# konstantineder/montecarlo-risk-engine

Measured on AMD Instinct MI355X. Metric: path-steps/sec at 1M paths x 250 steps; PV/CVA rel-error vs CPU ref, higher is better.
Workload: dtype f64

## Files before the change

### montecarlo-risk-engine_amd/csrc/kf_lean.hip

```cpp
#include <cstdlib>
#include <map>
#include <utility>

#include "kf_common.h"

namespace {

template <int NSLOT, int PPL>
__device__ __forceinline__ void lean_date_cva(const FastDateCvaLds* __restrict__ rp, const double (&reg)[PPL][2 * NSLOT], double (&cva)[PPL],
                                              const double* __restrict__ etab)
{
    const mcx_expq_coef ec = mcx_expq_load(mcx_region_zero());
    const FastDateCvaLds r = *rp;
    double xe[2 * PPL], ev[2 * PPL];
#pragma unroll
    for (int q = 0; q < PPL; ++q) {
        xe[2 * q] = fma(r.m_s1, reg[q][FDC_S_REG], fma(r.m_n1, reg[q][FDC_NI_REG], r.m_c0));
        xe[2 * q + 1] = fma(r.c_c1, reg[q][FDC_C_REG], r.c_c0);
    }
    mcx_exp_tab_n<2 * PPL>(xe, ev, etab, ec);
#pragma unroll
    for (int q = 0; q < PPL; ++q) {
        const double x = fma(r.x_d, reg[q][FDC_X_REG], r.x_a);
        double p = 0.0;
// ... 121 lines not shown
        const double r2 = fma(ed[q], -2.0 * 6.93147180559945309417e-01, tc[q].y) + fma(s * s, p, s);
        const double r = mcx_sqrt_gp(r2);
        const double sn = fma(sc[q].x, pc[q], sc[q].y * ps[q]);
        const double cs = fma(-sc[q].x, ps[q], sc[q].y * pc[q]);
        z0[q] = r * cs;
        z1[q] = r * sn;
        top = w1[q] > top ? w1[q] : top;
    }
    return top == 0xffffffffu;
}

#define MCX_LEAN_WAVES 4
template <int NSLOT, int NZ, bool INJECT, int SIG, int PPL, bool SIMULATE, int DK = 0>
__global__ __launch_bounds__(MCX_BLOCK, MCX_LEAN_WAVES) void kf_lean(const FusedArgs)
{
    static_assert(DK == 0 || (SIG == SIG_VAS_CIR_E && SIMULATE && !INJECT), "the cva-date kernel simulates the Vasicek + CIR++ signature");
    constexpr int NREG = 2 * NSLOT;
    constexpr int TILE = MCX_BLOCK * PPL;
    extern __shared__ double lds[];
    KArgs& a0 = kargs_region(0);
    const int n_rec = a0.n_rec;
    const int64_t n = a0.k1.n;
    for (int q = threadIdx.x; q < 9 * n_rec; q += MCX_BLOCK) lds[q] = 0.0;
    FastDateCvaLds* const dlds = (FastDateCvaLds*)(lds + ((9 * n_rec + 1) & ~1));
    if constexpr (DK != 0) {
        const FastDateCva* __restrict__ dc = a0.cva_dates;
        const double* __restrict__ cf = a0.coeffs;
        const int n_dates = a0.n_dates;
        for (int q = threadIdx.x; q < 16 * n_dates; q += MCX_BLOCK) {
            const int t = q >> 4, e = q & 15;
            double v;
            if (e < FDC_HEAD) {
                v = ((const double*)(dc + t))[e];
            } else {
                const int off = e < FDC_HEAD + 3 ? dc[t].coeff_off0 : dc[t].coeff_off1;
                v = off >= 0 ? cf[off + (e - FDC_HEAD) % 3] : 0.0;
            }
            ((double*)dlds)[q] = v;
        }
    }
    constexpr int BMB = SIG == SIG_VAS_CIR_E ? 10 : 7;
    constexpr int BM = (INJECT || !SIMULATE) ? 0 : MCX_BM_LDS_DOUBLES_B(BMB);
    __shared__ double tab_lds[BM + MCX_EXP_LDS_DOUBLES];
    const double* tab = nullptr;
    const double* etab = tab_lds + BM;
    mcx_exp_tab_load(tab_lds + BM);
    if (BM) { mcx_bm_load<BMB>(tab_lds); tab = tab_lds; }
    __syncthreads();
    const int64_t tiles = (n + TILE - 1) / TILE;
    double n_block = 0.0;

    for (int64_t tile = blockIdx.x; tile < tiles; tile += gridDim.x) {
        const bool first_tile = tile == (int64_t)blockIdx.x;
        int64_t i[PPL];
        bool live[PPL];
        uint64_t path[PPL];
        double reg[PPL][NREG];
        double cfs[PPL], cva[PPL];
        int est[PPL];
        int n_init, n_steps;
        {
            KArgs& a = kargs_region(mcx_region_zero());
            const auto& k = a.k1;
#pragma unroll
            for (int q = 0; q < PPL; ++q) {
                const int64_t i_raw = tile * TILE + q * MCX_BLOCK + threadIdx.x;
                live[q] = i_raw < n;
                i[q] = live[q] ? i_raw : n - 1;
                path[q] = k.path_offset + (uint64_t)i[q];
                sim_init_state<NSLOT, SIG>(k, reg[q]);
                cfs[q] = 0.0; cva[q] = 0.0;
                est[q] = a.init_state[0];
            }
            const int64_t rest = n - tile * TILE;
            n_block += (double)(rest < TILE ? rest : TILE);
            n_init = k.n_initial_store; n_steps = k.n_steps;
        }
        if (SIMULATE) {
        int step = 0, t_init = 0;
#pragma unroll 1
        while (true) {
            const bool init = t_init < n_init;
            if (!init && step >= n_steps) break;
            int st = init ? t_init : -1;
            t_init += init ? 1 : 0;
            {
                const int zr0 = mcx_region_zero();
                const auto& k = kargs_region(zr0).k1;
                const uint64_t seed = k.seed;
                const mcx_bm_coef bc = mcx_bm_coef_load(zr0);
                const mcx_bm_vconst vc = mcx_bm_vconst_make<BMB>(bc);
                uint32_t path_hi = 0;
                CvaDrawConst dc = {};
                if constexpr (DK == 1) { path_hi = ((const MCX_KONST uint32_t*)&k.path_offset)[1]; dc = cva_draw_const_make(); }
#pragma unroll 1
                while (st < 0 && step < n_steps) {
                    if constexpr (SIG == SIG_GENERIC) {
#pragma unroll
                        for (int q = 0; q < PPL; ++q) sim_substep<NSLOT, NZ, INJECT, SIG, BMB, true>(k, step, path[q], i[q], reg[q], tab, seed, bc, &vc);
                        st = ldk(&k.steps[step].store_idx);
                    } else {
                        double zz[PPL][NZ], uu[PPL];
                        bool rare = false;
                        const StepData<NSLOT, NZ> sdat = sim_step_load<NSLOT, NZ, SIG>(k, step);
                        __builtin_amdgcn_sched_barrier(0);
                        if constexpr (INJECT) {
#pragma unroll
                            for (int q = 0; q < PPL; ++q) sim_draw<NZ, true, SIG, BMB>(k, step, path[q], i[q], zz[q], uu[q], tab, seed, bc, &vc);
                        } else if constexpr (DK == 1) {
// ... 52 lines not shown
            load_row(n_dates > 1 ? 1 : 0, bufb);
#pragma unroll 1
            for (int t = 0; t < n_dates; t += 2) {
                lean_date<NSLOT, SIG, PPL, false>(t, i, live, first_tile, lds, reg, cfs, cva, est, etab);
                if (t + 2 < n_dates) load_row(t + 2, reg);
                if (t + 1 < n_dates) {
                    lean_date<NSLOT, SIG, PPL, false>(t + 1, i, live, first_tile, lds, bufb, cfs, cva, est, etab);
                    if (t + 3 < n_dates) load_row(t + 3, bufb);
                }
            }
        }
        {
            KArgs& a = kargs_region(mcx_region_zero());
#pragma unroll
            for (int q = 0; q < PPL; ++q) if (a.cfs && live[q]) a.cfs[i[q]] = cfs[q];
            if (a.rec_pv[0] >= 0) lean_record<PPL>(cfs, live, a.rec_pv[0], n_rec, first_tile, lds);
            if (a.rec_cva[0] >= 0) {
                const double lgd = a.lgd[0];
                double cc[PPL];
#pragma unroll
                for (int q = 0; q < PPL; ++q) cc[q] = cva[q] * lgd;
                lean_record<PPL>(cc, live, a.rec_cva[0], n_rec, first_tile, lds);
            }
        }
    }
    __syncthreads();
    for (int r = threadIdx.x; r < n_rec; r += MCX_BLOCK) {
        double s1 = 0.0, s2 = 0.0;
        for (int w = 0; w < 4; ++w) { s1 += lds[n_rec + (w * n_rec + r) * 2]; s2 += lds[n_rec + (w * n_rec + r) * 2 + 1]; }
        double* dst = a0.partials + ((int64_t)blockIdx.x * n_rec + r) * 4;
        dst[0] = n_block; dst[1] = lds[r]; dst[2] = s1; dst[3] = s2;
    }
}

template <int NSLOT, int NZ, int SIG, int PPL>
int launch_lean_shape(const FusedArgs& a, int full_steps, int n_cu, bool inject, bool simulate, hipStream_t s)
{
// ... 20 lines not shown
    if (!simulate) {
        auto kern = kf_lean<NSLOT, NZ, false, SIG, PPL, false>;
        grid = sized(residency(kern, lds));
        hipLaunchKernelGGL(kern, dim3(grid), dim3(MCX_BLOCK), lds, s, a);
    } else if (inject) {
        auto kern = kf_lean<NSLOT, NZ, true, SIG, PPL, true>;
        grid = sized(residency(kern, lds));
        hipLaunchKernelGGL(kern, dim3(grid), dim3(MCX_BLOCK), lds, s, a);
    } else {
        auto kern = kf_lean<NSLOT, NZ, false, SIG, PPL, true>;
        const int64_t resident = residency(kern, lds);
        if constexpr (SIG == SIG_VAS_CIR_E) {
            auto kern_cva = kf_lean<NSLOT, NZ, false, SIG, 2, true, 1>;
            auto kern_cva_thin = kf_lean<NSLOT, NZ, false, SIG, PPL, true, 2>;
            const bool one_high_word = ((a.k1.path_offset + (uint64_t)(a.k1.n - 1)) >> 32) == (a.k1.path_offset >> 32);
            if (a.cva_dates && one_high_word) {
                grid = sized(resident);
                if (PPL == 2 && grid >= resident) {
                    if (residency(kern_cva, lds_cva) >= resident) {
                        hipLaunchKernelGGL(kern_cva, dim3(grid), dim3(MCX_BLOCK), lds_cva, s, a);
                        return grid;
                    }
                } else if (residency(kern_cva_thin, lds_cva) >= resident) {
                    hipLaunchKernelGGL(kern_cva_thin, dim3(grid), dim3(MCX_BLOCK), lds_cva, s, a);
                    return grid;
                }
            }
        }
        grid = sized(resident);
        FusedArgs g = a;
        g.k1.n_steps = full_steps;
// ... 40 lines not shown
```

### montecarlo-risk-engine_amd/csrc/mcx_math.h

```cpp
#pragma once

__device__ const double MCX_EXP_C[14] __attribute__((aligned(64))) = {1.00000000000000000e+00, 1.00000000000000000e+00, 5.00000000000000000e-01, 1.66666666666666657e-01, 4.16666666666666644e-02, 8.33333333333333322e-03, 1.38888888888888894e-03, 1.98412698412698413e-04, 2.48015873015873016e-05, 2.75573192239858925e-06, 2.75573192239858883e-07, 2.50521083854417202e-08, 2.08767569878681002e-09, 1.60590438368216133e-10};
__device__ const double MCX_SIN_C[10] = {3.14159265358979312e+00, -5.16771278004997026e+00, 2.55016403987734552e+00, -5.99264529320792105e-01, 8.21458866111282326e-02, -7.37043094571435044e-03, 4.66302805767612554e-04, -2.19153534478302173e-05, 7.95205400147551261e-07, -2.29484289972698730e-08};
__device__ const double MCX_COS_C[10] = {1.00000000000000000e+00, -4.93480220054467900e+00, 4.05871212641676848e+00, -1.33526276885458950e+00, 2.35330630358893206e-01, -2.58068913900140612e-02, 1.92957430940392314e-03, -1.04638104924845705e-04, 4.30306958703294729e-06, -1.38789524622137714e-07};
__device__ const double MCX_LOG_C[7] = {6.666666666666735130e-01, 3.999999999940941908e-01, 2.857142874366239149e-01, 2.222219843214978396e-01, 1.818357216161805012e-01, 1.531383769920937332e-01, 1.479819860511658591e-01};

__device__ __forceinline__ int mcx_region_zero()
{
    int z;
    asm volatile("s_mov_b32 %0, 0" : "=s"(z));
    return z;
}
__device__ __forceinline__ uint32_t mcx_region_copy(uint32_t v)
{
    uint32_t o;
    asm volatile("s_mov_b32 %0, %1" : "=s"(o) : "s"(v));
    return o;
}

struct mcx_exp_coef { double c[14]; };
__device__ __forceinline__ mcx_exp_coef mcx_exp_load(int z = 0)
{
    return ldk_struct((const mcx_exp_coef*)(MCX_EXP_C + z));
}
// ... 104 lines not shown

__device__ __forceinline__ double mcx_sqrt_gp(double a)
{
    const double y = __builtin_amdgcn_rsq(a);
    const double g = a * y;
    const double h = 0.5 * y;
    return fma(g, fma(-h, g, 0.5), g);
}

#include "mcx_tables.h"
#define MCX_BM_LDS_DOUBLES_B(BMB) (4 << (BMB))
#define MCX_BM_LDS_DOUBLES MCX_BM_LDS_DOUBLES_B(7)
template <int BMB> struct mcx_bm_shape;
template <> struct mcx_bm_shape<7> {
    static constexpr int LOG_TERMS = 6, TRIG_TERMS = 3;
    static __device__ __forceinline__ double log_src(int q) { return MCX_LOG_TAB[q]; }
    static __device__ __forceinline__ double trig_src(int q) { return MCX_TRIG_TAB[q]; }
};
template <> struct mcx_bm_shape<10> {
    static constexpr int LOG_TERMS = 4, TRIG_TERMS = 2;
    static __device__ __forceinline__ double log_src(int q) { return MCX_LOG_TAB_L[q]; }
    static __device__ __forceinline__ double trig_src(int q) { return MCX_TRIG_TAB_L[q]; }
};

__device__ const double MCX_BM_C[12] __attribute__((aligned(64))) = {0.25, (1.0 / 3.0) * 0.25, 0.03125, 0.2 * 0.0625, (1.0 / 6.0) * 0.03125, (1.0 / 7.0) * 0.015625,
                                                                     -1.0 / 6.0, 1.0 / 120.0, -1.0 / 5040.0, -0.5, 1.0 / 24.0, -1.0 / 720.0};
struct mcx_bm_coef { double c[12]; };
__device__ __forceinline__ mcx_bm_coef mcx_bm_coef_load(int z = 0)
{
    return ldk_struct((const mcx_bm_coef*)(MCX_BM_C + z));
}

struct mcx_bm_vconst {
    double c54;
    double s53, s32;
    double log_head;
    double sin_head, cos_head;
    double trig_off;
};
__device__ __forceinline__ double mcx_opaque_v(double x) { asm volatile("" : "+v"(x)); return x; }
__device__ __forceinline__ double mcx_opaque_s(double x) { asm volatile("" : "+s"(x)); return x; }
template <int BMB = 7>
__device__ __forceinline__ mcx_bm_vconst mcx_bm_vconst_make(const mcx_bm_coef& C)
{
    using SH = mcx_bm_shape<BMB>;
    mcx_bm_vconst v;
    v.c54 = mcx_opaque_v(0x1.0p-54); v.s53 = mcx_opaque_s(0x1.0p-53); v.s32 = mcx_opaque_s(0x1.0p-32);
    v.log_head = mcx_opaque_v(C.c[SH::LOG_TERMS - 1]);
    v.sin_head = mcx_opaque_v(C.c[5 + SH::TRIG_TERMS]);
    v.cos_head = mcx_opaque_v(C.c[8 + SH::TRIG_TERMS]);
    v.trig_off = mcx_opaque_v(-3.14159265358979323846 / (double)(1 << BMB));
    return v;
}

template <int BMB = 7>
__device__ __forceinline__ void mcx_bm_load(double* __restrict__ tab)
{
    constexpr int N = 1 << BMB;
    for (int q = threadIdx.x; q < 2 * N; q += blockDim.x) {
        tab[q] = -2.0 * mcx_bm_shape<BMB>::log_src(q);
        tab[2 * N + q] = mcx_bm_shape<BMB>::trig_src(q);
    }
    __syncthreads();
}

typedef double mcx_d2 __attribute__((ext_vector_type(2)));

template <int BMB = 7>
__device__ __forceinline__ double mcx_m2log_tab(double x, const double* __restrict__ tab, const mcx_bm_coef& C, const mcx_bm_vconst* vc = nullptr)
{
    constexpr int N = 1 << BMB, LOG_TERMS = mcx_bm_shape<BMB>::LOG_TERMS;
    const double m = __builtin_amdgcn_frexp_mant(x);
    const int e = __builtin_amdgcn_frexp_exp(x);
    const int j = (__double2hiint(m) >> (20 - BMB)) & (N - 1);
    const mcx_d2 tc = ((const mcx_d2*)tab)[j];
    const double s = fma(m, tc.x, 2.0);
    double q = vc ? vc->log_head : C.c[LOG_TERMS - 1];
#pragma unroll
    for (int k = LOG_TERMS - 2; k >= 0; --k) q = fma(q, s, C.c[k]);
    const double p = fma(s * s, q, s);
    return fma((double)e, -2.0 * 6.93147180559945309417e-01, tc.y) + p;
// ... 19 lines not shown
    const double pc = fma(d2, qc, 1.0);
    s = fma(sc.x, pc, sc.y * ps);
    c = fma(-sc.x, ps, sc.y * pc);
}

#define MCX_EXP_LDS_DOUBLES 128
__device__ const double MCX_EXPQ_C[4] __attribute__((aligned(32))) = {0.5, 1.0 / 6.0, 1.0 / 24.0, 1.0 / 120.0};
struct mcx_expq_coef { double c[4]; };
__device__ __forceinline__ mcx_expq_coef mcx_expq_load(int z = 0) { return ldk_struct((const mcx_expq_coef*)(MCX_EXPQ_C + z)); }

__device__ __forceinline__ void mcx_exp_tab_load(double* __restrict__ tab)
{
    for (int q = threadIdx.x; q < MCX_EXP_LDS_DOUBLES; q += blockDim.x) tab[q] = MCX_EXP2_TAB[q];
}

__device__ __forceinline__ double mcx_exp_tab(double x, const double* __restrict__ tab, const mcx_expq_coef& C)
{
    const double k = rint(x * MCX_128_LN2);
    double r = fma(k, -MCX_LN2_128_HI, x);
    r = fma(k, -MCX_LN2_128_LO, r);
    const int ki = (int)k;
    const double T = tab[ki & 127];
    double q = fma(C.c[3], r, C.c[2]);
    q = fma(q, r, C.c[1]);
    q = fma(q, r, C.c[0]);
    q = fma(q, r, 1.0);
    q *= r;
    return ldexp(fma(T, q, T), ki >> 7);
}

// ... 27 lines not shown
```

### montecarlo-risk-engine_amd/csrc/mcx_tables.h

```cpp
#pragma once
__device__ const double MCX_LOG_TAB[256] = {
    0x1.fe01fe01fe020p+0, -0x1.60e52f45788e4p-1, 0x1.fa11caa01fa12p+0, -0x1.5ced1e17c35c6p-1,
    0x1.f6310aca0dbb5p+0, -0x1.58fcddce004c3p-1, 0x1.f25f644230ab5p+0, -0x1.55144fdbcbd62p-1,
    0x1.ee9c7f8458e02p+0, -0x1.513356667fc57p-1, 0x1.eae807aba01ebp+0, -0x1.4d59d43fdaba2p-1,
    0x1.e741aa59750e4p+0, -0x1.4987ace0dabb0p-1, 0x1.e3a9179dc1a73p+0, -0x1.45bcc464c893ap-1,
    0x1.e01e01e01e01ep+0, -0x1.41f8ff8471d61p-1, 0x1.dca01dca01dcap+0, -0x1.3e3c43918f76cp-1,
    0x1.d92f2231e7f8ap+0, -0x1.3a86767257112p-1, 0x1.d5cac807572b2p+0, -0x1.36d77e9d34fd7p-1,
    0x1.d272ca3fc5b1ap+0, -0x1.332f4314ad795p-1, 0x1.cf26e5c44bfc6p+0, -0x1.2f8dab6363379p-1,
    0x1.cbe6d9601cbe7p+0, -0x1.2bf29f9841c3bp-1, 0x1.c8b265afb8a42p+0, -0x1.285e0842ca384p-1,
    0x1.c5894d10d4986p+0, -0x1.24cfce6f80d9bp-1, 0x1.c26b5392ea01cp+0, -0x1.2147dba47a393p-1,
    0x1.bf583ee868d8bp+0, -0x1.1dc619de06944p-1, 0x1.bc4fd65883e7bp+0, -0x1.1a4a738b7a33cp-1,
    0x1.b951e2b18ff23p+0, -0x1.16d4d38c119fap-1, 0x1.b65e2e3beee05p+0, -0x1.1365252bf0865p-1,
    0x1.b37484ad806cep+0, -0x1.0ffb54213a476p-1, 0x1.b094b31d922a4p+0, -0x1.0c974c89431cep-1,
    0x1.adbe87f94905ep+0, -0x1.0938fae5d8e9bp-1, 0x1.aaf1d2f87ebfdp+0, -0x1.05e04c1aa2c06p-1,
    0x1.a82e65130e159p+0, -0x1.028d2d6a963f5p-1, 0x1.a574107688a4ap+0, -0x1.fe7f18eb03d3ep-2,
    0x1.a2c2a87c51ca0p+0, -0x1.f7eeae6b5761cp-2, 0x1.a01a01a01a01ap+0, -0x1.f168f7fb05c52p-2,
    0x1.9d79f176b682dp+0, -0x1.eaedd2eac990cp-2, 0x1.9ae24ea5510dap+0, -0x1.e47d1d32e677dp-2,
    0x1.9852f0d8ec0ffp+0, -0x1.de16b56ef90f0p-2, 0x1.95cbb0be377aep+0, -0x1.d7ba7ad9e7da1p-2,
    0x1.934c67f9b2ce6p+0, -0x1.d1684d49f46aep-2, 0x1.90d4f120190d5p+0, -0x1.cb200d2ceb643p-2,
    0x1.8e6527af1373fp+0, -0x1.c4e19b84723c2p-2, 0x1.8bfce8062ff3ap+0, -0x1.beacd9e271ad1p-2,
    0x1.899c0f601899cp+0, -0x1.b881aa659bc93p-2, 0x1.87427bcc092b9p+0, -0x1.b25fefb60cb2ep-2,
    0x1.84f00c2780614p+0, -0x1.ac478d0205070p-2, 0x1.82a4a0182a4a0p+0, -0x1.a63865fabd0ecp-2,
    0x1.8060180601806p+0, -0x1.a0325ed14fda4p-2, 0x1.7e225515a4f1dp+0, -0x1.9a355c33bd6bap-2,
    0x1.7beb3922e017cp+0, -0x1.9441434a0325ap-2, 0x1.79baa6bb6398bp+0, -0x1.8e55f9b349b82p-2,
// ... 27 lines not shown
    0x1.1ecf43c7fb84cp+0, -0x1.d179788219362p-4, 0x1.1d8f5672e4abdp+0, -0x1.bf968769fca18p-4,
    0x1.1c522fc1ce059p+0, -0x1.adc77ee5aea8ep-4, 0x1.1b17c67f2bae3p+0, -0x1.9c0c32d4d254dp-4,
    0x1.19e0119e0119ep+0, -0x1.8a6477a91dc29p-4, 0x1.18ab083902bdbp+0, -0x1.78d02263d82d7p-4,
    0x1.1778a191bd684p+0, -0x1.674f089365a78p-4, 0x1.1648d50fc3201p+0, -0x1.55e10050e0382p-4,
    0x1.151b9a3fdd5c9p+0, -0x1.4485e03dbdfb0p-4, 0x1.13f0e8d344724p+0, -0x1.333d7f8183f4ap-4,
    0x1.12c8b89edc0acp+0, -0x1.2207b5c7854a1p-4, 0x1.11a3019a74826p+0, -0x1.10e45b3cae829p-4,
    0x1.107fbbe011080p+0, -0x1.ffa6911ab9309p-5, 0x1.0f5edfab325a2p+0, -0x1.dda8adc67ee59p-5,
    0x1.0e40655826011p+0, -0x1.bbcebfc68f424p-5, 0x1.0d24456359e3ap+0, -0x1.9a187b573de81p-5,
    0x1.0c0a7868b4171p+0, -0x1.788595a3577c8p-5, 0x1.0af2f722eecb5p+0, -0x1.5715c4c03cee1p-5,
    0x1.09ddba6af8360p+0, -0x1.35c8bfaa13069p-5, 0x1.08cabb37565e2p+0, -0x1.149e3e4005a8dp-5,
    0x1.07b9f29b8eae2p+0, -0x1.e72bf2813ce6ap-6, 0x1.06ab59c7912fbp+0, -0x1.a55f548c5c427p-6,
    0x1.059eea0727586p+0, -0x1.63d6178690bbep-6, 0x1.04949cc1664c5p+0, -0x1.228fb1fea2e0ap-6,
    0x1.038c6b78247fcp+0, -0x1.c317384c75f0dp-7, 0x1.02864fc7729e9p+0, -0x1.41929f968330cp-7,
    0x1.0182436517a37p+0, -0x1.8121214586b02p-8, 0x1.0000000000000p+0, 0.0,
};
__device__ const double MCX_TRIG_TAB[256] = {
    0x1.92155f7a3667ep-6, 0x1.ffd886084cd0dp-1, 0x1.2d52092ce19f6p-4, 0x1.fe9cdad01883ap-1,
    0x1.f564e56a9730ep-4, 0x1.fc26470e19fd3p-1, 0x1.5e214448b3fc6p-3, 0x1.f8764fa714ba9p-1,
    0x1.c0b826a7e4f63p-3, 0x1.f38f3ac64e589p-1, 0x1.111d262b1f677p-2, 0x1.ed740e7684963p-1,
    0x1.4135c94176601p-2, 0x1.e6288ec48e112p-1, 0x1.7088530fa459fp-2, 0x1.ddb13b6ccc23cp-1,
    0x1.9ef7943a8ed8ap-2, 0x1.d4134d14dc93ap-1, 0x1.cc66e9931c45ep-2, 0x1.c954b213411f5p-1,
    0x1.f8ba4dbf89abap-2, 0x1.bd7c0ac6f952ap-1, 0x1.11eb3541b4b23p-1, 0x1.b090a58150200p-1,
    0x1.26d054cdd12dfp-1, 0x1.a29a7a0462782p-1, 0x1.3affa292050b9p-1, 0x1.93a22499263fbp-1,
    0x1.4e6cabbe3e5e9p-1, 0x1.83b0e0bff976ep-1, 0x1.610b7551d2cdfp-1, 0x1.72d0837efff96p-1,
    0x1.72d0837efff96p-1, 0x1.610b7551d2cdfp-1, 0x1.83b0e0bff976ep-1, 0x1.4e6cabbe3e5e9p-1,
    0x1.93a22499263fbp-1, 0x1.3affa292050b9p-1, 0x1.a29a7a0462782p-1, 0x1.26d054cdd12dfp-1,
    0x1.b090a58150200p-1, 0x1.11eb3541b4b23p-1, 0x1.bd7c0ac6f952ap-1, 0x1.f8ba4dbf89abap-2,
    0x1.c954b213411f5p-1, 0x1.cc66e9931c45ep-2, 0x1.d4134d14dc93ap-1, 0x1.9ef7943a8ed8ap-2,
    0x1.ddb13b6ccc23cp-1, 0x1.7088530fa459fp-2, 0x1.e6288ec48e112p-1, 0x1.4135c94176601p-2,
    0x1.ed740e7684963p-1, 0x1.111d262b1f677p-2, 0x1.f38f3ac64e589p-1, 0x1.c0b826a7e4f63p-3,
    0x1.f8764fa714ba9p-1, 0x1.5e214448b3fc6p-3, 0x1.fc26470e19fd3p-1, 0x1.f564e56a9730ep-4,
// ... 35 lines not shown
    -0x1.f38f3ac64e589p-1, 0x1.c0b826a7e4f63p-3, -0x1.ed740e7684963p-1, 0x1.111d262b1f677p-2,
    -0x1.e6288ec48e112p-1, 0x1.4135c94176601p-2, -0x1.ddb13b6ccc23cp-1, 0x1.7088530fa459fp-2,
    -0x1.d4134d14dc93ap-1, 0x1.9ef7943a8ed8ap-2, -0x1.c954b213411f5p-1, 0x1.cc66e9931c45ep-2,
    -0x1.bd7c0ac6f952ap-1, 0x1.f8ba4dbf89abap-2, -0x1.b090a58150200p-1, 0x1.11eb3541b4b23p-1,
    -0x1.a29a7a0462782p-1, 0x1.26d054cdd12dfp-1, -0x1.93a22499263fbp-1, 0x1.3affa292050b9p-1,
    -0x1.83b0e0bff976ep-1, 0x1.4e6cabbe3e5e9p-1, -0x1.72d0837efff96p-1, 0x1.610b7551d2cdfp-1,
    -0x1.610b7551d2cdfp-1, 0x1.72d0837efff96p-1, -0x1.4e6cabbe3e5e9p-1, 0x1.83b0e0bff976ep-1,
    -0x1.3affa292050b9p-1, 0x1.93a22499263fbp-1, -0x1.26d054cdd12dfp-1, 0x1.a29a7a0462782p-1,
    -0x1.11eb3541b4b23p-1, 0x1.b090a58150200p-1, -0x1.f8ba4dbf89abap-2, 0x1.bd7c0ac6f952ap-1,
    -0x1.cc66e9931c45ep-2, 0x1.c954b213411f5p-1, -0x1.9ef7943a8ed8ap-2, 0x1.d4134d14dc93ap-1,
    -0x1.7088530fa459fp-2, 0x1.ddb13b6ccc23cp-1, -0x1.4135c94176601p-2, 0x1.e6288ec48e112p-1,
    -0x1.111d262b1f677p-2, 0x1.ed740e7684963p-1, -0x1.c0b826a7e4f63p-3, 0x1.f38f3ac64e589p-1,
    -0x1.5e214448b3fc6p-3, 0x1.f8764fa714ba9p-1, -0x1.f564e56a9730ep-4, 0x1.fc26470e19fd3p-1,
    -0x1.2d52092ce19f6p-4, 0x1.fe9cdad01883ap-1, -0x1.92155f7a3667ep-6, 0x1.ffd886084cd0dp-1,
};
__device__ const double MCX_LOG_TAB_L[2048] = {
    0x1.ffc007ff00200p+0, -0x1.62a433ef4e51ap-1, 0x1.ff4047e50a1c3p+0, -0x1.622453e6a6263p-1,
    0x1.fec0c7834def5p+0, -0x1.61a493c60c729p-1, 0x1.fe4186aa2b1a5p+0, -0x1.6124f37d991d4p-1,
    0x1.fdc2852a30896p+0, -0x1.60a572fd6fef1p-1, 0x1.fd43c2d41c590p+0, -0x1.60261235c0874p-1,
    0x1.fcc53f78db9b2p+0, -0x1.5fa6d116c64f7p-1, 0x1.fc46fae98a1d1p+0, -0x1.5f27af90c8705p-1,
    0x1.fbc8f4f7722d6p+0, -0x1.5ea8ad9419c5bp-1, 0x1.fb4b2d740c629p+0, -0x1.5e29cb1118d32p-1,
    0x1.facda430ff61ap+0, -0x1.5dab07f82fb84p-1, 0x1.fa5059001fa50p+0, -0x1.5d2c6439d4252p-1,
    0x1.f9d34bb36f445p+0, -0x1.5caddfc6874f5p-1, 0x1.f9567c1d1dbbap+0, -0x1.5c2f7a8ed5e5bp-1,
    0x1.f8d9ea0f87b41p+0, -0x1.5bb1348358064p-1, 0x1.f85d955d36cbbp+0, -0x1.5b330d94b131ap-1,
    0x1.f7e17dd8e15e6p+0, -0x1.5ab505b39040bp-1, 0x1.f765a3556a4eep+0, -0x1.5a371cd0af592p-1,
    0x1.f6ea05a5e0d04p+0, -0x1.59b952dcd3e28p-1, 0x1.f66ea49d802f2p+0, -0x1.593ba7c8ce7adp-1,
    0x1.f5f3800faf9c0p+0, -0x1.58be1b857aebep-1, 0x1.f57897d001f58p+0, -0x1.5840ae03c0204p-1,
    0x1.f4fdebb23592ap+0, -0x1.57c35f3490183p-1, 0x1.f4837b8a340e3p+0, -0x1.57462f08e7df5p-1,
    0x1.f409472c12115p+0, -0x1.56c91d71cf810p-1, 0x1.f38f4e6c0f1f9p+0, -0x1.564c2a6059fe7p-1,
    0x1.f315911e95625p+0, -0x1.55cf55c5a5437p-1, 0x1.f29c0f1839750p+0, -0x1.55529f92da1c2p-1,
    0x1.f222c82dba316p+0, -0x1.54d607b92c29dp-1, 0x1.f1a9bc34007c7p+0, -0x1.54598e29d9d95p-1,
// ... 483 lines not shown
    0x1.037bfa2bf7218p+0, -0x1.bafb16b749182p-7, 0x1.035b1dd2ca3dfp+0, -0x1.aac45e026ca43p-7,
    0x1.033a49cb37c1cp+0, -0x1.9a8fb2d091f35p-7, 0x1.03197e121767bp+0, -0x1.8a5d149cb8a0bp-7,
    0x1.02f8baa442836p+0, -0x1.7a2c82e212c55p-7, 0x1.02d7ff7e94004p+0, -0x1.69fdfd1c04d7ap-7,
    0x1.02b74c9de8608p+0, -0x1.59d182c6258adp-7, 0x1.0296a1ff1dbc3p+0, -0x1.49a7135c3dc5dp-7,
    0x1.0275ff9f13c02p+0, -0x1.397eae5a487a4p-7, 0x1.0255657aabad0p+0, -0x1.2958533c729a5p-7,
    0x1.0234d38ec8564p+0, -0x1.1934017f1aef7p-7, 0x1.021449d84e212p+0, -0x1.0911b89ed207ap-7,
    0x1.01f3c8542303dp+0, -0x1.f1e2f030b4562p-8, 0x1.01d34eff2e845p+0, -0x1.d1a67ed14e623p-8,
    0x1.01b2ddd659b76p+0, -0x1.b16e1c19bcbacp-8, 0x1.019274d68f3fdp+0, -0x1.9139c704acd81p-8,
    0x1.017213fcbb4d4p+0, -0x1.71097e8d2eac3p-8, 0x1.0151bb45cb9b4p+0, -0x1.50dd41aeb48a9p-8,
    0x1.01316aaeaf705p+0, -0x1.30b50f6512ef5p-8, 0x1.01112234579d1p+0, -0x1.1090e6ac8075ap-8,
    0x1.00f0e1d3b67b1p+0, -0x1.e0e18d032adbcp-9, 0x1.00d0a989bfebfp+0, -0x1.a0a95bc297863p-9,
    0x1.00b0795369587p+0, -0x1.60793791fd9f1p-9, 0x1.0090512da9af7p+0, -0x1.20511e6cd6419p-9,
    0x1.0070311579652p+0, -0x1.c0621c9eb9adfp-10, 0x1.00501907d271cp+0, -0x1.40320a6d1c38ep-10,
    0x1.00300901b0511p+0, -0x1.80240480a21ecp-11, 0x1.0000000000000p+0, 0.0,
};
__device__ const double MCX_TRIG_TAB_L[2048] = {
    0x1.921f8becca4bap-9, 0x1.ffff621621d02p-1, 0x1.2d96b0e509703p-7, 0x1.fffa72c978c4fp-1,
    0x1.f6a296ab997cbp-7, 0x1.fff0943c53bd1p-1, 0x1.5fd4d21fab226p-6, 0x1.ffe1c6870cb77p-1,
    0x1.c454f4ce53b1dp-6, 0x1.ffce09ce2a679p-1, 0x1.14685db42c17fp-5, 0x1.ffb55e425fdaep-1,
    0x1.46a396ff86179p-5, 0x1.ff97c4208c014p-1, 0x1.78dbaa5874686p-5, 0x1.ff753bb1b9164p-1,
    0x1.ab101bd5f8317p-5, 0x1.ff4dc54b1bed3p-1, 0x1.dd406f9808ec9p-5, 0x1.ff21614e131edp-1,
    0x1.07b614e463064p-4, 0x1.fef0102826191p-1, 0x1.20c9674ed444dp-4, 0x1.feb9d2530410fp-1,
    0x1.39d9f12c5a299p-4, 0x1.fe7ea85482d60p-1, 0x1.52e774a4d4d0ap-4, 0x1.fe3e92be9d886p-1,
    0x1.6bf1b3e79b129p-4, 0x1.fdf9922f73307p-1, 0x1.84f8712c130a1p-4, 0x1.fdafa7514538cp-1,
    0x1.9dfb6eb24a85cp-4, 0x1.fd60d2da75c9ep-1, 0x1.b6fa6ec38f64cp-4, 0x1.fd0d158d86087p-1,
    0x1.cff533b307dc1p-4, 0x1.fcb4703914354p-1, 0x1.e8eb7fde4aa3fp-4, 0x1.fc56e3b7d9af6p-1,
    0x1.00ee8ad6fb85bp-3, 0x1.fbf470f0a8d88p-1, 0x1.0d64dbcb26786p-3, 0x1.fb8d18d66adb7p-1,
    0x1.19d8940be24e7p-3, 0x1.fb20dc681d54dp-1, 0x1.264994dfd3409p-3, 0x1.faafbcb0cfddcp-1,
    0x1.32b7bf94516a7p-3, 0x1.fa39bac7a1791p-1, 0x1.3f22f57db4893p-3, 0x1.f9bed7cfbde29p-1,
    0x1.4b8b17f79fa88p-3, 0x1.f93f14f85ac08p-1, 0x1.57f008654cbdep-3, 0x1.f8ba737cb4b78p-1,
    0x1.6451a831d830dp-3, 0x1.f830f4a40c60cp-1, 0x1.70afd8d08c4ffp-3, 0x1.f7a299c1a322ap-1,
// ... 483 lines not shown
    -0x1.57f008654cbdep-3, 0x1.f8ba737cb4b78p-1, -0x1.4b8b17f79fa88p-3, 0x1.f93f14f85ac08p-1,
    -0x1.3f22f57db4893p-3, 0x1.f9bed7cfbde29p-1, -0x1.32b7bf94516a7p-3, 0x1.fa39bac7a1791p-1,
    -0x1.264994dfd3409p-3, 0x1.faafbcb0cfddcp-1, -0x1.19d8940be24e7p-3, 0x1.fb20dc681d54dp-1,
    -0x1.0d64dbcb26786p-3, 0x1.fb8d18d66adb7p-1, -0x1.00ee8ad6fb85bp-3, 0x1.fbf470f0a8d88p-1,
    -0x1.e8eb7fde4aa3fp-4, 0x1.fc56e3b7d9af6p-1, -0x1.cff533b307dc1p-4, 0x1.fcb4703914354p-1,
    -0x1.b6fa6ec38f64cp-4, 0x1.fd0d158d86087p-1, -0x1.9dfb6eb24a85cp-4, 0x1.fd60d2da75c9ep-1,
    -0x1.84f8712c130a1p-4, 0x1.fdafa7514538cp-1, -0x1.6bf1b3e79b129p-4, 0x1.fdf9922f73307p-1,
    -0x1.52e774a4d4d0ap-4, 0x1.fe3e92be9d886p-1, -0x1.39d9f12c5a299p-4, 0x1.fe7ea85482d60p-1,
    -0x1.20c9674ed444dp-4, 0x1.feb9d2530410fp-1, -0x1.07b614e463064p-4, 0x1.fef0102826191p-1,
    -0x1.dd406f9808ec9p-5, 0x1.ff21614e131edp-1, -0x1.ab101bd5f8317p-5, 0x1.ff4dc54b1bed3p-1,
    -0x1.78dbaa5874686p-5, 0x1.ff753bb1b9164p-1, -0x1.46a396ff86179p-5, 0x1.ff97c4208c014p-1,
    -0x1.14685db42c17fp-5, 0x1.ffb55e425fdaep-1, -0x1.c454f4ce53b1dp-6, 0x1.ffce09ce2a679p-1,
    -0x1.5fd4d21fab226p-6, 0x1.ffe1c6870cb77p-1, -0x1.f6a296ab997cbp-7, 0x1.fff0943c53bd1p-1,
    -0x1.2d96b0e509703p-7, 0x1.fffa72c978c4fp-1, -0x1.921f8becca4bap-9, 0x1.ffff621621d02p-1,
};
__device__ const double MCX_EXP2_TAB[128] = {
    0x1.0000000000000p+0, 0x1.0163da9fb3335p+0, 0x1.02c9a3e778061p+0, 0x1.04315e86e7f85p+0,
    0x1.059b0d3158574p+0, 0x1.0706b29ddf6dep+0, 0x1.0874518759bc8p+0, 0x1.09e3ecac6f383p+0,
    0x1.0b5586cf9890fp+0, 0x1.0cc922b7247f7p+0, 0x1.0e3ec32d3d1a2p+0, 0x1.0fb66affed31bp+0,
    0x1.11301d0125b51p+0, 0x1.12abdc06c31ccp+0, 0x1.1429aaea92de0p+0, 0x1.15a98c8a58e51p+0,
    0x1.172b83c7d517bp+0, 0x1.18af9388c8deap+0, 0x1.1a35beb6fcb75p+0, 0x1.1bbe084045cd4p+0,
    0x1.1d4873168b9aap+0, 0x1.1ed5022fcd91dp+0, 0x1.2063b88628cd6p+0, 0x1.21f49917ddc96p+0,
    0x1.2387a6e756238p+0, 0x1.251ce4fb2a63fp+0, 0x1.26b4565e27cddp+0, 0x1.284dfe1f56381p+0,
    0x1.29e9df51fdee1p+0, 0x1.2b87fd0dad990p+0, 0x1.2d285a6e4030bp+0, 0x1.2ecafa93e2f56p+0,
    0x1.306fe0a31b715p+0, 0x1.32170fc4cd831p+0, 0x1.33c08b26416ffp+0, 0x1.356c55f929ff1p+0,
    0x1.371a7373aa9cbp+0, 0x1.38cae6d05d866p+0, 0x1.3a7db34e59ff7p+0, 0x1.3c32dc313a8e5p+0,
    0x1.3dea64c123422p+0, 0x1.3fa4504ac801cp+0, 0x1.4160a21f72e2ap+0, 0x1.431f5d950a897p+0,
    0x1.44e086061892dp+0, 0x1.46a41ed1d0057p+0, 0x1.486a2b5c13cd0p+0, 0x1.4a32af0d7d3dep+0,
    0x1.4bfdad5362a27p+0, 0x1.4dcb299fddd0dp+0, 0x1.4f9b2769d2ca7p+0, 0x1.516daa2cf6642p+0,
    0x1.5342b569d4f82p+0, 0x1.551a4ca5d920fp+0, 0x1.56f4736b527dap+0, 0x1.58d12d497c7fdp+0,
    0x1.5ab07dd485429p+0, 0x1.5c9268a5946b7p+0, 0x1.5e76f15ad2148p+0, 0x1.605e1b976dc09p+0,
// ... 22 lines not shown
```

Baseline: 308.2 billion.

## Overlap kernel prologue table and CVA-date loads, hoist per-run constants per tile

Rewrites the kernel prologue so the Box-Muller tables, the exp2 table and the per-date CVA descriptors are fetched into registers with wide, aligned vector loads. Explicit waitcnt fences let these global loads overlap with each other before a single LDS store pass. The per-run draw constants (seed, coefficients, vconst) are computed once per tile for the CVA-date kernels instead of on every run entry. Scale constants are kept in VGPRs for the thin kernel, and a host-side guard restricts the CVA kernel to argument-initialised state layouts. This cuts prologue latency and loop-entry overhead, at the cost of more register pressure and reliance on hand-placed wait counts.

After: 318.1 billion (median of 6 runs). 3.2% higher.

```diff
diff --git a/montecarlo-risk-engine_amd/csrc/kf_lean.hip b/montecarlo-risk-engine_amd/csrc/kf_lean.hip
--- a/montecarlo-risk-engine_amd/csrc/kf_lean.hip
+++ b/montecarlo-risk-engine_amd/csrc/kf_lean.hip
@@ -159,7 +159,7 @@
 template <int NSLOT, int NZ, bool INJECT, int SIG, int PPL, bool SIMULATE, int DK = 0>
 __global__ __launch_bounds__(MCX_BLOCK, MCX_LEAN_WAVES) void kf_lean(const FusedArgs)
 {
-    static_assert(DK == 0 || (SIG == SIG_VAS_CIR_E && SIMULATE && !INJECT), "the cva-date kernel simulates the Vasicek + CIR++ signature");
+    static_assert(DK == 0 || (SIG == SIG_VAS_CIR_E && SIMULATE && !INJECT && NSLOT == 2), "the cva-date kernel simulates the Vasicek + CIR++ signature");
     constexpr int NREG = 2 * NSLOT;
     constexpr int TILE = MCX_BLOCK * PPL;
     extern __shared__ double lds[];
@@ -168,29 +168,63 @@
     const int64_t n = a0.k1.n;
     for (int q = threadIdx.x; q < 9 * n_rec; q += MCX_BLOCK) lds[q] = 0.0;
     FastDateCvaLds* const dlds = (FastDateCvaLds*)(lds + ((9 * n_rec + 1) & ~1));
-    if constexpr (DK != 0) {
-        const FastDateCva* __restrict__ dc = a0.cva_dates;
-        const double* __restrict__ cf = a0.coeffs;
-        const int n_dates = a0.n_dates;
-        for (int q = threadIdx.x; q < 16 * n_dates; q += MCX_BLOCK) {
-            const int t = q >> 4, e = q & 15;
-            double v;
-            if (e < FDC_HEAD) {
-                v = ((const double*)(dc + t))[e];
-            } else {
-                const int off = e < FDC_HEAD + 3 ? dc[t].coeff_off0 : dc[t].coeff_off1;
-                v = off >= 0 ? cf[off + (e - FDC_HEAD) % 3] : 0.0;
-            }
-            ((double*)dlds)[q] = v;
-        }
-    }
     constexpr int BMB = SIG == SIG_VAS_CIR_E ? 10 : 7;
     constexpr int BM = (INJECT || !SIMULATE) ? 0 : MCX_BM_LDS_DOUBLES_B(BMB);
-    __shared__ double tab_lds[BM + MCX_EXP_LDS_DOUBLES];
+    __shared__ double tab_lds[BM + MCX_EXP_LDS_DOUBLES] __attribute__((aligned(16)));
     const double* tab = nullptr;
     const double* etab = tab_lds + BM;
-    mcx_exp_tab_load(tab_lds + BM);
-    if (BM) { mcx_bm_load<BMB>(tab_lds); tab = tab_lds; }
+    constexpr int VM_LANDED = 0x0F70;
+    constexpr int FDC_ROUNDS = 4, FDC_STRIDE = MCX_BLOCK / 16;
+    typedef int mcx_i2 __attribute__((ext_vector_type(2)));
+    static_assert(MCX_BLOCK % 16 == 0 && offsetof(FastDateCva, coeff_off1) == offsetof(FastDateCva, coeff_off0) + 4, "one lane, one field");
+    const int n_dates = DK != 0 ? a0.n_dates : 0;
+    const int fdc_e = threadIdx.x & 15, fdc_t0 = threadIdx.x >> 4;
+    const bool fdc_head = fdc_e < FDC_HEAD;
+    auto fdc_round1 = [&](int base, mcx_i2 (&h)[FDC_ROUNDS]) {
+        const FastDateCva* __restrict__ dc = a0.cva_dates;
+        const int src = fdc_head ? 8 * fdc_e : (int)offsetof(FastDateCva, coeff_off0);
+#pragma unroll
+        for (int r = 0; r < FDC_ROUNDS; ++r) {
+            const int t = base + r * FDC_STRIDE + fdc_t0;
+            h[r] = *(const mcx_i2*)((const char*)(dc + (t < n_dates ? t : n_dates - 1)) + src);
+        }
+    };
+    mcx_i2 fdc_h[FDC_ROUNDS] = {};
+    if (DK != 0 && n_dates > 0) fdc_round1(0, fdc_h);
+    mcx_bm_regs<BMB, MCX_BLOCK> bmr;
+    if constexpr (BM != 0) bmr = mcx_bm_fetch<BMB, MCX_BLOCK>();
+    const double exr = mcx_exp_tab_fetch<MCX_BLOCK>();
+    if constexpr (DK != 0) {
+        const double* __restrict__ cf = a0.coeffs;
+        const int row_e = (fdc_e - FDC_HEAD) % 3;
+#pragma unroll 1
+        for (int base = 0; base < n_dates; base += FDC_ROUNDS * FDC_STRIDE) {
+            double v[FDC_ROUNDS];
+            __builtin_amdgcn_sched_barrier(0);
+            __builtin_amdgcn_s_waitcnt(VM_LANDED);
+            __builtin_amdgcn_sched_barrier(0);
+#pragma unroll
+            for (int r = 0; r < FDC_ROUNDS; ++r) {
+                const int off = fdc_e < FDC_HEAD + 3 ? fdc_h[r].x : fdc_h[r].y;
+                v[r] = __hiloint2double(fdc_h[r].y, fdc_h[r].x);
+                if (!fdc_head) v[r] = off >= 0 ? cf[off + row_e] : 0.0;
+            }
+            fdc_round1(base + FDC_ROUNDS * FDC_STRIDE, fdc_h);
+            __builtin_amdgcn_sched_barrier(0);
+            __builtin_amdgcn_s_waitcnt(VM_LANDED);
+            __builtin_amdgcn_sched_barrier(0);
+#pragma unroll
+            for (int r = 0; r < FDC_ROUNDS; ++r) {
+                const int t = base + r * FDC_STRIDE + fdc_t0;
+                if (t < n_dates) ((double*)dlds)[16 * t + fdc_e] = v[r];
+            }
+        }
+    }
+    __builtin_amdgcn_sched_barrier(0);
+    __builtin_amdgcn_s_waitcnt(VM_LANDED);
+    __builtin_amdgcn_sched_barrier(0);
+    mcx_exp_tab_store(tab_lds + BM, exr);
+    if constexpr (BM != 0) { mcx_bm_store<BMB, MCX_BLOCK>(tab_lds, bmr); tab = tab_lds; }
     __syncthreads();
     const int64_t tiles = (n + TILE - 1) / TILE;
     double n_block = 0.0;
@@ -213,7 +247,12 @@
                 live[q] = i_raw < n;
                 i[q] = live[q] ? i_raw : n - 1;
                 path[q] = k.path_offset + (uint64_t)i[q];
-                sim_init_state<NSLOT, SIG>(k, reg[q]);
+                if constexpr (DK != 0) {
+#pragma unroll
+                    for (int j = 0; j < NREG; ++j) reg[q][j] = k.init_state[j];
+                } else {
+                    sim_init_state<NSLOT, SIG>(k, reg[q]);
+                }
                 cfs[q] = 0.0; cva[q] = 0.0;
                 est[q] = a.init_state[0];
             }
@@ -221,6 +260,31 @@
             n_block += (double)(rest < TILE ? rest : TILE);
             n_init = k.n_initial_store; n_steps = k.n_steps;
         }
+        struct RunEntry {
+            int zr;
+            uint64_t seed;
+            mcx_bm_coef bc;
+            mcx_bm_vconst vc;
+            uint32_t path_hi;
+            CvaDrawConst dc;
+        };
+        auto run_entry = [](int zr0) {
+            RunEntry e;
+            e.zr = zr0;
+            const auto& k = kargs_region(zr0).k1;
+            e.seed = k.seed;
+            e.bc = mcx_bm_coef_load(zr0);
+            e.vc = mcx_bm_vconst_make<BMB, DK == 2 && PPL == 1>(e.bc);
+            if constexpr (DK == 2 && PPL == 1) {
+#pragma unroll
+                for (int q = 0; q < 12; ++q) asm("" : "+v"(e.bc.c[q]));
+            }
+            e.path_hi = 0; e.dc = CvaDrawConst{};
+            if constexpr (DK == 1) { e.path_hi = ((const MCX_KONST uint32_t*)&k.path_offset)[1]; e.dc = cva_draw_const_make(); }
+            return e;
+        };
+        RunEntry tile_entry = {};
+        if constexpr (DK != 0 && SIMULATE) tile_entry = run_entry(mcx_region_zero());
         if (SIMULATE) {
         int step = 0, t_init = 0;
 #pragma unroll 1
@@ -230,14 +294,13 @@
             int st = init ? t_init : -1;
             t_init += init ? 1 : 0;
             {
-                const int zr0 = mcx_region_zero();
-                const auto& k = kargs_region(zr0).k1;
-                const uint64_t seed = k.seed;
-                const mcx_bm_coef bc = mcx_bm_coef_load(zr0);
-                const mcx_bm_vconst vc = mcx_bm_vconst_make<BMB>(bc);
-                uint32_t path_hi = 0;
-                CvaDrawConst dc = {};
-                if constexpr (DK == 1) { path_hi = ((const MCX_KONST uint32_t*)&k.path_offset)[1]; dc = cva_draw_const_make(); }
+                const RunEntry re = DK != 0 ? tile_entry : run_entry(mcx_region_zero());
+                const auto& k = kargs_region(re.zr).k1;
+                const uint64_t seed = re.seed;
+                const mcx_bm_coef& bc = re.bc;
+                const mcx_bm_vconst& vc = re.vc;
+                const uint32_t path_hi = re.path_hi;
+                const CvaDrawConst& dc = re.dc;
 #pragma unroll 1
                 while (st < 0 && step < n_steps) {
                     if constexpr (SIG == SIG_GENERIC) {
@@ -320,13 +383,14 @@
             KArgs& a = kargs_region(mcx_region_zero());
 #pragma unroll
             for (int q = 0; q < PPL; ++q) if (a.cfs && live[q]) a.cfs[i[q]] = cfs[q];
-            if (a.rec_pv[0] >= 0) lean_record<PPL>(cfs, live, a.rec_pv[0], n_rec, first_tile, lds);
+            const int n_rec_e = a.n_rec;
+            if (a.rec_pv[0] >= 0) lean_record<PPL>(cfs, live, a.rec_pv[0], n_rec_e, first_tile, lds);
             if (a.rec_cva[0] >= 0) {
                 const double lgd = a.lgd[0];
                 double cc[PPL];
 #pragma unroll
                 for (int q = 0; q < PPL; ++q) cc[q] = cva[q] * lgd;
-                lean_record<PPL>(cc, live, a.rec_cva[0], n_rec, first_tile, lds);
+                lean_record<PPL>(cc, live, a.rec_cva[0], n_rec_e, first_tile, lds);
             }
         }
     }
@@ -377,7 +441,8 @@
             auto kern_cva = kf_lean<NSLOT, NZ, false, SIG, 2, true, 1>;
             auto kern_cva_thin = kf_lean<NSLOT, NZ, false, SIG, PPL, true, 2>;
             const bool one_high_word = ((a.k1.path_offset + (uint64_t)(a.k1.n - 1)) >> 32) == (a.k1.path_offset >> 32);
-            if (a.cva_dates && one_high_word) {
+            const bool arg_state = !a.k1.init_paths && a.k1.slots[0].state_off == 0 && a.k1.slots[1].state_off == 2;
+            if (a.cva_dates && one_high_word && arg_state) {
                 grid = sized(resident);
                 if (PPL == 2 && grid >= resident) {
                     if (residency(kern_cva, lds_cva) >= resident) {
diff --git a/montecarlo-risk-engine_amd/csrc/mcx_math.h b/montecarlo-risk-engine_amd/csrc/mcx_math.h
--- a/montecarlo-risk-engine_amd/csrc/mcx_math.h
+++ b/montecarlo-risk-engine_amd/csrc/mcx_math.h
@@ -142,13 +142,13 @@
 template <int BMB> struct mcx_bm_shape;
 template <> struct mcx_bm_shape<7> {
     static constexpr int LOG_TERMS = 6, TRIG_TERMS = 3;
-    static __device__ __forceinline__ double log_src(int q) { return MCX_LOG_TAB[q]; }
-    static __device__ __forceinline__ double trig_src(int q) { return MCX_TRIG_TAB[q]; }
+    static __device__ __forceinline__ const double& log_src(int q) { return MCX_LOG_TAB[q]; }
+    static __device__ __forceinline__ const double& trig_src(int q) { return MCX_TRIG_TAB[q]; }
 };
 template <> struct mcx_bm_shape<10> {
     static constexpr int LOG_TERMS = 4, TRIG_TERMS = 2;
-    static __device__ __forceinline__ double log_src(int q) { return MCX_LOG_TAB_L[q]; }
-    static __device__ __forceinline__ double trig_src(int q) { return MCX_TRIG_TAB_L[q]; }
+    static __device__ __forceinline__ const double& log_src(int q) { return MCX_LOG_TAB_L[q]; }
+    static __device__ __forceinline__ const double& trig_src(int q) { return MCX_TRIG_TAB_L[q]; }
 };
 
 __device__ const double MCX_BM_C[12] __attribute__((aligned(64))) = {0.25, (1.0 / 3.0) * 0.25, 0.03125, 0.2 * 0.0625, (1.0 / 6.0) * 0.03125, (1.0 / 7.0) * 0.015625,
@@ -168,12 +168,14 @@
 };
 __device__ __forceinline__ double mcx_opaque_v(double x) { asm volatile("" : "+v"(x)); return x; }
 __device__ __forceinline__ double mcx_opaque_s(double x) { asm volatile("" : "+s"(x)); return x; }
-template <int BMB = 7>
+template <int BMB = 7, bool SCALE_V = false>
 __device__ __forceinline__ mcx_bm_vconst mcx_bm_vconst_make(const mcx_bm_coef& C)
 {
     using SH = mcx_bm_shape<BMB>;
     mcx_bm_vconst v;
-    v.c54 = mcx_opaque_v(0x1.0p-54); v.s53 = mcx_opaque_s(0x1.0p-53); v.s32 = mcx_opaque_s(0x1.0p-32);
+    v.c54 = mcx_opaque_v(0x1.0p-54);
+    if constexpr (SCALE_V) { v.s53 = mcx_opaque_v(0x1.0p-53); v.s32 = mcx_opaque_v(0x1.0p-32); }
+    else { v.s53 = mcx_opaque_s(0x1.0p-53); v.s32 = mcx_opaque_s(0x1.0p-32); }
     v.log_head = mcx_opaque_v(C.c[SH::LOG_TERMS - 1]);
     v.sin_head = mcx_opaque_v(C.c[5 + SH::TRIG_TERMS]);
     v.cos_head = mcx_opaque_v(C.c[8 + SH::TRIG_TERMS]);
@@ -193,6 +195,41 @@
 }
 
 typedef double mcx_d2 __attribute__((ext_vector_type(2)));
+
+template <int BMB, int BLOCK>
+struct mcx_bm_regs {
+    static constexpr int N = 1 << BMB, ROUNDS = (N + BLOCK - 1) / BLOCK;
+    mcx_d2 lg[ROUNDS], tr[ROUNDS];
+};
+template <int BMB, int BLOCK>
+__device__ __forceinline__ mcx_bm_regs<BMB, BLOCK> mcx_bm_fetch()
+{
+    using R = mcx_bm_regs<BMB, BLOCK>;
+    R v;
+#pragma unroll
+    for (int r = 0; r < R::ROUNDS; ++r) {
+        const int q = r * BLOCK + (int)threadIdx.x;
+        v.lg[r] = v.tr[r] = mcx_d2{0.0, 0.0};
+        if (R::N % BLOCK == 0 || q < R::N) {
+            v.lg[r] = *(const mcx_d2*)&mcx_bm_shape<BMB>::log_src(2 * q);
+            v.tr[r] = *(const mcx_d2*)&mcx_bm_shape<BMB>::trig_src(2 * q);
+        }
+    }
+    return v;
+}
+template <int BMB, int BLOCK>
+__device__ __forceinline__ void mcx_bm_store(double* __restrict__ tab, const mcx_bm_regs<BMB, BLOCK>& v)
+{
+    using R = mcx_bm_regs<BMB, BLOCK>;
+#pragma unroll
+    for (int r = 0; r < R::ROUNDS; ++r) {
+        const int q = r * BLOCK + (int)threadIdx.x;
+        if (R::N % BLOCK == 0 || q < R::N) {
+            ((mcx_d2*)tab)[q] = mcx_d2{-2.0 * v.lg[r].x, -2.0 * v.lg[r].y};
+            ((mcx_d2*)(tab + 2 * R::N))[q] = v.tr[r];
+        }
+    }
+}
 
 template <int BMB = 7>
 __device__ __forceinline__ double mcx_m2log_tab(double x, const double* __restrict__ tab, const mcx_bm_coef& C, const mcx_bm_vconst* vc = nullptr)
@@ -242,6 +279,17 @@
     for (int q = threadIdx.x; q < MCX_EXP_LDS_DOUBLES; q += blockDim.x) tab[q] = MCX_EXP2_TAB[q];
 }
 
+template <int BLOCK>
+__device__ __forceinline__ double mcx_exp_tab_fetch()
+{
+    static_assert(BLOCK >= MCX_EXP_LDS_DOUBLES && (MCX_EXP_LDS_DOUBLES & (MCX_EXP_LDS_DOUBLES - 1)) == 0, "one entry per lane");
+    return MCX_EXP2_TAB[threadIdx.x & (MCX_EXP_LDS_DOUBLES - 1)];
+}
+__device__ __forceinline__ void mcx_exp_tab_store(double* __restrict__ tab, double v)
+{
+    if (threadIdx.x < MCX_EXP_LDS_DOUBLES) tab[threadIdx.x] = v;
+}
+
 __device__ __forceinline__ double mcx_exp_tab(double x, const double* __restrict__ tab, const mcx_expq_coef& C)
 {
     const double k = rint(x * MCX_128_LN2);
diff --git a/montecarlo-risk-engine_amd/csrc/mcx_tables.h b/montecarlo-risk-engine_amd/csrc/mcx_tables.h
--- a/montecarlo-risk-engine_amd/csrc/mcx_tables.h
+++ b/montecarlo-risk-engine_amd/csrc/mcx_tables.h
@@ -1,5 +1,5 @@
 #pragma once
-__device__ const double MCX_LOG_TAB[256] = {
+__device__ const double MCX_LOG_TAB[256] __attribute__((aligned(16))) = {
     0x1.fe01fe01fe020p+0, -0x1.60e52f45788e4p-1, 0x1.fa11caa01fa12p+0, -0x1.5ced1e17c35c6p-1,
     0x1.f6310aca0dbb5p+0, -0x1.58fcddce004c3p-1, 0x1.f25f644230ab5p+0, -0x1.55144fdbcbd62p-1,
     0x1.ee9c7f8458e02p+0, -0x1.513356667fc57p-1, 0x1.eae807aba01ebp+0, -0x1.4d59d43fdaba2p-1,
@@ -65,7 +65,7 @@
     0x1.038c6b78247fcp+0, -0x1.c317384c75f0dp-7, 0x1.02864fc7729e9p+0, -0x1.41929f968330cp-7,
     0x1.0182436517a37p+0, -0x1.8121214586b02p-8, 0x1.0000000000000p+0, 0.0,
 };
-__device__ const double MCX_TRIG_TAB[256] = {
+__device__ const double MCX_TRIG_TAB[256] __attribute__((aligned(16))) = {
     0x1.92155f7a3667ep-6, 0x1.ffd886084cd0dp-1, 0x1.2d52092ce19f6p-4, 0x1.fe9cdad01883ap-1,
     0x1.f564e56a9730ep-4, 0x1.fc26470e19fd3p-1, 0x1.5e214448b3fc6p-3, 0x1.f8764fa714ba9p-1,
     0x1.c0b826a7e4f63p-3, 0x1.f38f3ac64e589p-1, 0x1.111d262b1f677p-2, 0x1.ed740e7684963p-1,
@@ -131,7 +131,7 @@
     -0x1.5e214448b3fc6p-3, 0x1.f8764fa714ba9p-1, -0x1.f564e56a9730ep-4, 0x1.fc26470e19fd3p-1,
     -0x1.2d52092ce19f6p-4, 0x1.fe9cdad01883ap-1, -0x1.92155f7a3667ep-6, 0x1.ffd886084cd0dp-1,
 };
-__device__ const double MCX_LOG_TAB_L[2048] = {
+__device__ const double MCX_LOG_TAB_L[2048] __attribute__((aligned(16))) = {
     0x1.ffc007ff00200p+0, -0x1.62a433ef4e51ap-1, 0x1.ff4047e50a1c3p+0, -0x1.622453e6a6263p-1,
     0x1.fec0c7834def5p+0, -0x1.61a493c60c729p-1, 0x1.fe4186aa2b1a5p+0, -0x1.6124f37d991d4p-1,
     0x1.fdc2852a30896p+0, -0x1.60a572fd6fef1p-1, 0x1.fd43c2d41c590p+0, -0x1.60261235c0874p-1,
@@ -645,7 +645,7 @@
     0x1.0070311579652p+0, -0x1.c0621c9eb9adfp-10, 0x1.00501907d271cp+0, -0x1.40320a6d1c38ep-10,
     0x1.00300901b0511p+0, -0x1.80240480a21ecp-11, 0x1.0000000000000p+0, 0.0,
 };
-__device__ const double MCX_TRIG_TAB_L[2048] = {
+__device__ const double MCX_TRIG_TAB_L[2048] __attribute__((aligned(16))) = {
     0x1.921f8becca4bap-9, 0x1.ffff621621d02p-1, 0x1.2d96b0e509703p-7, 0x1.fffa72c978c4fp-1,
     0x1.f6a296ab997cbp-7, 0x1.fff0943c53bd1p-1, 0x1.5fd4d21fab226p-6, 0x1.ffe1c6870cb77p-1,
     0x1.c454f4ce53b1dp-6, 0x1.ffce09ce2a679p-1, 0x1.14685db42c17fp-5, 0x1.ffb55e425fdaep-1,
@@ -1159,7 +1159,7 @@
     -0x1.5fd4d21fab226p-6, 0x1.ffe1c6870cb77p-1, -0x1.f6a296ab997cbp-7, 0x1.fff0943c53bd1p-1,
     -0x1.2d96b0e509703p-7, 0x1.fffa72c978c4fp-1, -0x1.921f8becca4bap-9, 0x1.ffff621621d02p-1,
 };
-__device__ const double MCX_EXP2_TAB[128] = {
+__device__ const double MCX_EXP2_TAB[128] __attribute__((aligned(16))) = {
     0x1.0000000000000p+0, 0x1.0163da9fb3335p+0, 0x1.02c9a3e778061p+0, 0x1.04315e86e7f85p+0,
     0x1.059b0d3158574p+0, 0x1.0706b29ddf6dep+0, 0x1.0874518759bc8p+0, 0x1.09e3ecac6f383p+0,
     0x1.0b5586cf9890fp+0, 0x1.0cc922b7247f7p+0, 0x1.0e3ec32d3d1a2p+0, 0x1.0fb66affed31bp+0,
```
